# sunwookim028/bwa-mem-gpu

Hardware: AMD Instinct MI355X
Metric: reads/s aligned (150 bp PE vs hg38-scale 3100 Mbp synthetic genome), file to file (bwahip_stream_run) (higher is better)
Workload: dtype u64

## Files before the change

### bwa-mem-gpu_amd/bwahip.py

```python
import ctypes as C
import os
import subprocess
import numpy as np

_HERE = os.path.dirname(os.path.abspath(__file__))
LIB_PATH = os.environ.get("BWAHIP_LIB") or os.path.join(_HERE, "libbwahip.so")
TOOLS = os.path.join(_HERE, "tools")


class Opt(C.Structure):
    _fields_ = [("max_mem_intv", C.c_uint64), ("a", C.c_int), ("b", C.c_int), ("o_del", C.c_int), ("e_del", C.c_int),
                ("o_ins", C.c_int), ("e_ins", C.c_int), ("pen_unpaired", C.c_int), ("pen_clip5", C.c_int),
                ("pen_clip3", C.c_int), ("w", C.c_int), ("zdrop", C.c_int), ("T", C.c_int), ("flag", C.c_int),
                ("min_seed_len", C.c_int), ("min_chain_weight", C.c_int), ("max_chain_extend", C.c_int),
                ("split_factor", C.c_float), ("split_width", C.c_int), ("max_occ", C.c_int), ("max_chain_gap", C.c_int),
                ("n_threads", C.c_int), ("chunk_size", C.c_int), ("mask_level", C.c_float), ("drop_ratio", C.c_float),
                ("XA_drop_ratio", C.c_float), ("mask_level_redun", C.c_float), ("mapQ_coef_len", C.c_float),
                ("mapQ_coef_fac", C.c_int), ("max_ins", C.c_int), ("max_matesw", C.c_int), ("max_XA_hits", C.c_int),
                ("max_XA_hits_alt", C.c_int), ("mat", C.c_int8 * 25)]


class Seq(C.Structure):
    _fields_ = [("l_seq", C.c_int), ("id", C.c_int), ("name", C.c_char_p), ("comment", C.c_char_p),
                ("seq", C.POINTER(C.c_char)), ("qual", C.c_char_p), ("sam", C.POINTER(C.c_char)),
# ... 1149 lines not shown
        return ["k_smem(passes 1-2)+k_smem_heavy+k_smem3(pass 3)+k_intv_sort", "k_seeds", "k_chain(+k_chain_big,k_chain_flt)", "k_seed_sw (only with -W / reads > 700 bp)",
                "k_extend_spec+k_extend(+k_extend_big, dedup/patch)", "pe_rescue = PE: k_pestat + k_pe_prepare + k_pe_copy (insert sizes, lists; the rescue kernels k_matesw_sw / k_matesw start on the second stream)",
                "k_mark (mark primary) + PE: k_pair (pairing) beside the rescue kernels, then both for the rescued pairs",
                "k_cigar (mem_reg2aln: mapQ, CIGAR by ksw_global2 backtrack, NM/MD)", "k_sam size + scan + write (SAM text)"]

    @staticmethod
    def output_description(paired):
        return "SAM text of the batch in HBM (== seqs[i].sam of mem_process_seqs, " + ("paired-end: mate rescue, pairing, paired records)" if paired else "single-end)")

    def counters(self):
        buf = (C.c_uint64 * 32)()
        _check(lib().bwahip_batch_counters(self._h, buf, 32), "bwahip_batch_counters")
        names = ["extend", "blocks", "sa", "lf", "intv", "seeds", "cells", "max_extends", "chain_build_max", "chain_sort_max", "chain_flt_max",
                 "chain_write_max", "max_seeds", "max_chains", "ext_max", "ext_dedup_max", "heavy_blocks", "heavy_intv", "heavy_reads",
                 "dp_rows_1col", "dp_rows_ncol", "dedup_sort1_max", "dedup_loop_max", "dedup_sort2_max",
                 "pass3_blocks", "pass3_intv", "pass3_jumped", "ext_calls", "ext_diag", "_29", "_30", "_31"]
        return {k: int(buf[i]) for i, k in enumerate(names)}

    def kat_introsort(self, k64, score, qb, mode):
        k64 = np.ascontiguousarray(k64, dtype=np.int64); score = np.ascontiguousarray(score, dtype=np.int32); qb = np.ascontiguousarray(qb, dtype=np.int32)
        n = len(k64)
        a = np.empty(n, dtype=np.int32); b = np.empty(n, dtype=np.int32); st = np.zeros(2, dtype=np.int32)
        _check(lib().bwahip_kat_introsort(self._h, n, mode, k64.ctypes.data, score.ctypes.data, qb.ctypes.data, a.ctypes.data, b.ctypes.data, st.ctypes.data), "bwahip_kat_introsort")
        assert st[1] == 0
        return a, b, bool(st[0])

    def kat_mate_insert(self, list_off, list_words, step_off, step_hit, step_words, opt=None, mode=0, where=0):
        opt = opt or default_opt()
        list_off = np.ascontiguousarray(list_off, dtype=np.int64); step_off = np.ascontiguousarray(step_off, dtype=np.int64)
        list_words = np.ascontiguousarray(list_words, dtype=np.int64).reshape(-1, 19); step_words = np.ascontiguousarray(step_words, dtype=np.int64).reshape(-1, 19)
        step_hit = np.ascontiguousarray(step_hit, dtype=np.int32)
# ... 311 lines not shown
```

### bwa-mem-gpu_amd/csrc/bwahip_internal.h

```cpp
#pragma once
#include <hip/hip_runtime.h>
#include <stdint.h>
#include <stdio.h>
#include <stdlib.h>
#include <string.h>
#include <vector>
#include <string>
#include "../../include/bwahip.h"

#define HIP_TRY(expr) do { hipError_t e_ = (expr); if (e_ != hipSuccess) { \
	fprintf(stderr, "[bwahip] %s failed at %s:%d: %s\n", #expr, __FILE__, __LINE__, hipGetErrorString(e_)); \
	return BWAHIP_ENODEV; } } while (0)

struct DevAnn { int64_t offset; int32_t len; int32_t is_alt; };

struct DevIndex {
	const uint4 *bwt;
	const uint64_t *sa;
	const uint8_t *pac;
	const DevAnn *anns;
	uint64_t primary, L2[5], seq_len, n_sa;
	int64_t l_pac;
	int sa_intv, sa_shift, n_seqs;
	const uint4 *kmer; int kmer_k;
// ... 1 lines not shown
__host__ __device__ inline uint64_t kmer_off(int L) { return (0x5555555555555555ull & ((1ull << 2 * L) - 1)) - 1; }

struct DevOpt {
	int a, b, o_del, e_del, o_ins, e_ins, pen_clip5, pen_clip3, w, zdrop;
	int min_seed_len, split_width, max_occ, max_chain_gap, max_mem_intv, split_len;
	int min_chain_weight, max_chain_extend;
	float mask_level, drop_ratio, mask_level_redun;
	int8_t mat[25];
	int T, flag, pen_unpaired, max_ins, max_matesw, max_XA_hits, max_XA_hits_alt, mapQ_coef_fac;
	float XA_drop_ratio, mapQ_coef_len;
};

enum { CNT_EXTEND = 0, CNT_BLOCKS, CNT_SA, CNT_LF, CNT_INTV, CNT_SEEDS, CNT_CELLS, CNT_MAX_EXT ,
       CNT_HEAVY_BLOCKS = 16, CNT_HEAVY_INTV, CNT_HEAVY_READS, CNT_ROWS1 , CNT_ROWSN ,
       CNT_P3_BLOCKS = 24, CNT_P3_INTV, CNT_P3_JUMPED ,
       CNT_EXT_CALLS , CNT_EXT_DIAG , CNT_N = 32 };
constexpr int CNT_SLOTS = 256;
#define BWAHIP_MISC_BYTES ((size_t)CNT_SLOTS * CNT_N * 8 + 64)
#ifdef __HIPCC__
__device__ __forceinline__ unsigned long long *cnt_row(unsigned long long *base)
{
	return base + (size_t)((blockIdx.x * (blockDim.x >> 6) + (threadIdx.x >> 6)) & (CNT_SLOTS - 1)) * CNT_N;
}
#endif

struct __attribute__((aligned(32))) DevIntv { uint64_t x0, x1, x2, info; };

struct __attribute__((aligned(16))) DevSeed { int64_t rbeg; int32_t qbeg, len; int32_t score, rid; };

struct DevChain {
	int64_t pos;
// ... 36 lines not shown
	DevIndex ix; DevOpt opt;
	int n_reads; const uint8_t *seq; const int64_t *off;
	uint64_t *seq4; int seq4_stride;
	DevIntv *out; int *out_n; int cap;
	DevIntv *raw; int *raw_n;
	int *seed_cnt;
	float *frac_rep_lrep;
	int *l_rep;
	DevIntv *scratch; int lcap;
	unsigned int *queue;
	unsigned long long *counters;
	int *err;
	int groups_total;
	int *worst_n;
	int *heavy_list; unsigned int *heavy_n; int heavy_mult;
};
int launch_smem(const SmemLaunch &a, int group_lanes, hipStream_t st);
int launch_pack4(const SmemLaunch &a, hipStream_t st);
int launch_smem_heavy(const SmemLaunch &a, hipStream_t st);
int launch_smem3(const SmemLaunch &a, hipStream_t st);
int launch_kmer_table(const DevIndex &ix, uint4 *tab, int K, hipStream_t st);
int launch_kmer_check(const DevIndex &ix, int L, unsigned long long *bad, hipStream_t st);
int launch_intv_sort(const SmemLaunch &a, hipStream_t st);
int smem_default_groups(int group_lanes);

struct SeedLaunch {
	DevIndex ix; DevOpt opt;
	int n_reads; const int64_t *off;
	const DevIntv *intv; const int *intv_n; int cap;
	const int64_t *seed_base;
// ... 204 lines not shown
```

### bwa-mem-gpu_amd/csrc/ctx_internal.h

```cpp
#pragma once
#include "bwahip_internal.h"
#include "own.h"
#include <atomic>
#include <memory>
#include <string>
#include <utility>

inline std::atomic<long> g_bwahip_reallocs{0};
inline std::atomic<int64_t> g_bwahip_live[6];

struct DevMem {
	static constexpr size_t slack = 256;
	static constexpr const char *what = "hipMalloc";
	static void *alloc(size_t bytes)
	{
		void *p = nullptr;
		if (hipMalloc(&p, bytes ? bytes : 1) != hipSuccess) { (void)hipGetLastError(); return nullptr; }
		++g_bwahip_live[0]; g_bwahip_live[1] += (int64_t)bytes;
		return p;
	}
	static void free(void *p, size_t bytes) { (void)hipFree(p); --g_bwahip_live[0]; g_bwahip_live[1] -= (int64_t)bytes; }
	static void count_sync() { ++g_bwahip_reallocs; }
};
struct PinnedMem {
// ... 38 lines not shown
	{
		reset();
		if (hipStreamCreateWithFlags(&s, flags) != hipSuccess) { (void)hipGetLastError(); s = nullptr; return BWAHIP_ENODEV; }
		++g_bwahip_live[5];
		return 0;
	}
	void reset() { if (s) { (void)hipStreamDestroy(s); --g_bwahip_live[5]; s = nullptr; } }
	operator hipStream_t() const { return s; }
};

struct Knobs {
	int intv_cap = 96;
	int smem_lanes = 1;
	int sa_intv = 1;
	int kmer_k = 14;
	int heavy_mult = -1;
	int chain_mid_max = 1536, chain_big_max = 3200, chain_glb_grid = 2048;
	int chain_big_min = 512;
	int rank_sort_min = 2;
	int spec_min_chains = 16;
	int ext_lds_window = 1 << 30;
	int ext_early_stop = 1;
	int ext_diag = 1;
	int sorted_piece_blocks = 1024;
	int gpu_final = 1;
	int gpu_pair = 1;
	int incr_insert = 1;
	int verbose = 0;
	int e2e_log = 0;
	const char *dump_ext = nullptr;
	void from_env()
	{
		auto geti = [](const char *k, int &v) { if (const char *e = getenv(k)) v = atoi(e); };
		geti("BWAHIP_INTV_CAP", intv_cap); geti("BWAHIP_SMEM_LANES", smem_lanes); geti("BWAHIP_HEAVY_MULT", heavy_mult); geti("BWAHIP_SA_INTV", sa_intv); geti("BWAHIP_KMER_K", kmer_k);
		geti("BWAHIP_CHAIN_BIG_MIN", chain_big_min); geti("BWAHIP_CHAIN_MID_MAX", chain_mid_max); geti("BWAHIP_CHAIN_BIG_MAX", chain_big_max); geti("BWAHIP_CHAIN_GLB_GRID", chain_glb_grid); geti("BWAHIP_RANK_SORT_MIN", rank_sort_min); geti("BWAHIP_SPEC_MIN_CHAINS", spec_min_chains); geti("BWAHIP_EXT_LDS_WINDOW", ext_lds_window); geti("BWAHIP_EXT_EARLY_STOP", ext_early_stop); geti("BWAHIP_EXT_DIAG", ext_diag); geti("BWAHIP_GPU_FINAL", gpu_final); geti("BWAHIP_GPU_PAIR", gpu_pair);
		verbose = getenv("BWAHIP_VERBOSE") != nullptr;
		e2e_log = getenv("BWAHIP_E2E_LOG") != nullptr;
		dump_ext = getenv("BWAHIP_DUMP_EXT");
		if (intv_cap < 2) intv_cap = 2;
		ext_early_stop = ext_early_stop != 0; ext_diag = ext_diag != 0;
		geti("BWAHIP_INCR_INSERT", incr_insert); incr_insert = incr_insert != 0;
		geti("BWAHIP_SORTED_PIECE_BLOCKS", sorted_piece_blocks);
		if (sorted_piece_blocks < 1 || sorted_piece_blocks > 4096) sorted_piece_blocks = 1024;
	}
};

struct BatchText {
	std::vector<int64_t> off, qoff, noff, coff;
	int64_t qtot = 0;
// ... 200 lines not shown
```

### bwa-mem-gpu_amd/csrc/fmi_dev.h

```cpp
#pragma once
#include "bwahip_internal.h"

__device__ __forceinline__ int lane_id() { return (int)(threadIdx.x & 63); }

template <int K> __device__ __forceinline__ uint32_t quad_bcast(uint32_t v)
{
	constexpr int ctrl = K | K << 2 | K << 4 | K << 6;
	return (uint32_t)__builtin_amdgcn_update_dpp(0, (int)v, ctrl, 0xf, 0xf, false);
}
template <int K> __device__ __forceinline__ uint64_t quad_bcast64(uint64_t v)
{
	return (uint64_t)quad_bcast<K>((uint32_t)v) | (uint64_t)quad_bcast<K>((uint32_t)(v >> 32)) << 32;
}
__device__ __forceinline__ uint32_t quad_xor1(uint32_t v) { return (uint32_t)__builtin_amdgcn_update_dpp(0, (int)v, 0xB1, 0xf, 0xf, false); }
__device__ __forceinline__ uint32_t quad_xor2(uint32_t v) { return (uint32_t)__builtin_amdgcn_update_dpp(0, (int)v, 0x4E, 0xf, 0xf, false); }
__device__ __forceinline__ uint32_t half_mirror(uint32_t v) { return (uint32_t)__builtin_amdgcn_update_dpp(0, (int)v, 0x141, 0xf, 0xf, false); }
__device__ __forceinline__ uint64_t half_mirror64(uint64_t v)
{
	return (uint64_t)half_mirror((uint32_t)v) | (uint64_t)half_mirror((uint32_t)(v >> 32)) << 32;
}

__device__ __forceinline__ uint32_t count_bases64(uint4 v, int n)
{
	const int n0 = n < 32 ? n : 32, n1 = n - n0;
// ... 127 lines not shown
	const bool none = (p == ~0ull);
	uint64_t pp = p - (p >= ix.primary);
	uint4 v0 = make_uint4(0, 0, 0, 0), v1 = v0, v2 = v0, v3 = v0;
	if (live && !none) {
		const uint4 *b = ix.bwt + (pp >> 7) * 4;
		v0 = b[0]; v1 = b[1]; v2 = b[2]; v3 = b[3];
	}
	const int o = (int)(pp & 127) + 1;
	const uint32_t packed = count_bases64(v2, o < 64 ? o : 64) + count_bases64(v3, o > 64 ? o - 64 : 0);
	cnt[0] = ((uint64_t)v0.y << 32 | v0.x) + (packed & 0xff);
	cnt[1] = ((uint64_t)v0.w << 32 | v0.z) + (packed >> 8 & 0xff);
	cnt[2] = ((uint64_t)v1.y << 32 | v1.x) + (packed >> 16 & 0xff);
	cnt[3] = ((uint64_t)v1.w << 32 | v1.z) + (packed >> 24);
	if (none) cnt[0] = cnt[1] = cnt[2] = cnt[3] = 0;
}
__device__ __forceinline__ void lane_occ4_pair(const DevIndex &ix, uint64_t pk, uint64_t pl, bool live, uint64_t ck[4], uint64_t cl[4])
{
	const bool nk = (pk == ~0ull);
	const uint64_t kk = pk - (pk >= ix.primary), ll = pl - (pl >= ix.primary);
	uint4 a0 = make_uint4(0, 0, 0, 0), a1 = a0, a2 = a0, a3 = a0;
	const bool same = !nk && (kk >> 7) == (ll >> 7);
	const bool k_hi = (kk & 127) >= 64, l_hi = (ll & 127) >= 64;
	if (live && !nk) { const uint4 *b = ix.bwt + (kk >> 7) * 4; a0 = b[0]; a1 = b[1]; a2 = b[2]; if (k_hi || (same && l_hi)) a3 = b[3]; }
	uint4 b0 = a0, b1 = a1, b2 = a2, b3 = a3;
	if (live && !same && pl != ~0ull) { const uint4 *b = ix.bwt + (ll >> 7) * 4; b0 = b[0]; b1 = b[1]; b2 = b[2]; if (l_hi) b3 = b[3]; }
	{
		const int o = (int)(kk & 127) + 1;
		const uint32_t packed = count_bases64(a2, o < 64 ? o : 64) + count_bases64(a3, o > 64 ? o - 64 : 0);
		ck[0] = ((uint64_t)a0.y << 32 | a0.x) + (packed & 0xff); ck[1] = ((uint64_t)a0.w << 32 | a0.z) + (packed >> 8 & 0xff);
		ck[2] = ((uint64_t)a1.y << 32 | a1.x) + (packed >> 16 & 0xff); ck[3] = ((uint64_t)a1.w << 32 | a1.z) + (packed >> 24);
		if (nk) ck[0] = ck[1] = ck[2] = ck[3] = 0;
	}
	{
		const int o = (int)(ll & 127) + 1;
		const uint32_t packed = count_bases64(b2, o < 64 ? o : 64) + count_bases64(b3, o > 64 ? o - 64 : 0);
		cl[0] = ((uint64_t)b0.y << 32 | b0.x) + (packed & 0xff); cl[1] = ((uint64_t)b0.w << 32 | b0.z) + (packed >> 8 & 0xff);
		cl[2] = ((uint64_t)b1.y << 32 | b1.x) + (packed >> 16 & 0xff); cl[3] = ((uint64_t)b1.w << 32 | b1.z) + (packed >> 24);
		if (pl == ~0ull) cl[0] = cl[1] = cl[2] = cl[3] = 0;
	}
}

__device__ __forceinline__ int lane_extend_c(const DevIndex &ix, const Bi &ik, int is_back, int c, bool live, Bi &o)
{
	uint64_t xa = is_back ? ik.x0 : ik.x1;
	uint64_t xb = is_back ? ik.x1 : ik.x0;
	uint64_t k = xa - 1, l = k + ik.x2;
	uint64_t tk[4], tl[4];
	lane_occ4_pair(ix, k, l, live, tk, tl);
	uint64_t s1 = tl[1] - tk[1], s2 = tl[2] - tk[2], s3 = tl[3] - tk[3];
	uint64_t lo = L2_at(ix, c) + 1 + sel4(c, tk[0], tk[1], tk[2], tk[3]);
	uint64_t sz = sel4(c, tl[0] - tk[0], s1, s2, s3);
	uint64_t cum = (c < 3 ? s3 : 0) + (c < 2 ? s2 : 0) + (c < 1 ? s1 : 0);
	uint64_t bb = xb + (xa <= ix.primary && xa + ik.x2 - 1 >= ix.primary) + cum;
	o.x0 = is_back ? lo : bb;
	o.x1 = is_back ? bb : lo;
	o.x2 = sz;
	if (!live) return 0;
	uint64_t kk = k - (k >= ix.primary), ll = l - (l >= ix.primary);
	return (k == ~0ull || (kk >> 7) != (ll >> 7)) ? 2 : 1;
}

__device__ __forceinline__ uint64_t pair_swap64(uint64_t v) { return (uint64_t)quad_xor1((uint32_t)v) | (uint64_t)quad_xor1((uint32_t)(v >> 32)) << 32; }
__device__ __forceinline__ int pair_extend_c(const DevIndex &ix, const Bi &ik, int is_back, int c, bool live, Bi &o)
// ... 68 lines not shown
```

### bwa-mem-gpu_amd/csrc/k_smem.hip

```cpp
#include "fmi_dev.h"

namespace {

enum : int { ST_IDLE = 0, ST_NEXT, ST_FWD, ST_BWD, ST_FINISH };

__device__ __forceinline__ void put(DevIntv *p, uint64_t x0, uint64_t x1, uint64_t x2, uint64_t info)
{
	ulonglong2 *q = reinterpret_cast<ulonglong2*>(p);
	q[0] = make_ulonglong2(x0, x1);
	q[1] = make_ulonglong2(x2, info);
}
__device__ __forceinline__ void get(const DevIntv *p, uint64_t &x0, uint64_t &x1, uint64_t &x2, uint64_t &info)
{
	const ulonglong2 *q = reinterpret_cast<const ulonglong2*>(p);
	ulonglong2 a = q[0], b = q[1];
	x0 = a.x; x1 = a.y; x2 = b.x; info = b.y;
}

__device__ __forceinline__ uint64_t get_info(const DevIntv *p) { return reinterpret_cast<const ulonglong2*>(p)[1].y; }
__device__ __forceinline__ uint64_t get_x2(const DevIntv *p) { return reinterpret_cast<const ulonglong2*>(p)[1].x; }

__device__ __forceinline__ uint4 pack_entry(uint64_t x0, uint64_t x1, uint64_t x2, uint32_t end)
{
	const uint32_t h0 = (uint32_t)(x0 >> 32), h1 = (uint32_t)(x1 >> 32), h2 = (uint32_t)(x2 >> 32);
// ... 1 lines not shown
}
__device__ __forceinline__ void unpack_entry(uint4 v, uint64_t &x0, uint64_t &x1, uint64_t &x2, uint64_t &end)
{
	x0 = (uint64_t)(v.w & 63) << 32 | v.x;
	x1 = (uint64_t)(v.w >> 6 & 63) << 32 | v.y;
	x2 = (uint64_t)(v.w >> 12 & 63) << 32 | v.z;
	end = v.w >> 18;
}

__device__ __forceinline__ int qbase(const uint64_t *row, int p, uint64_t &qw, int &qwi)
{
	const int wi = p >> 4;
	if (wi != qwi) { qw = row[wi]; qwi = wi; }
	const uint32_t half = (p & 8) ? (uint32_t)(qw >> 32) : (uint32_t)qw;
	return (int)(half >> ((p & 7) * 4)) & 15;
}

__global__ __launch_bounds__(256) void k_pack4(int n_reads, const uint8_t *seq, const int64_t *off, uint64_t *seq4, int stride)
{
	const int64_t t = (int64_t)blockIdx.x * blockDim.x + threadIdx.x;
	if (t >= (int64_t)n_reads * stride) return;
	const int r = (int)(t / stride), w = (int)(t % stride);
	const uint8_t *s = seq + off[r];
	const int len = (int)(off[r + 1] - off[r]);
	uint64_t v = 0;
	for (int k = 0; k < 16; ++k) {
		const int p = w * 16 + k;
		const uint64_t code = p < len ? (s[p] > 3 ? 4 : s[p]) : 15;
		v |= code << (4 * k);
	}
// ... 19 lines not shown
		if (x2 > (uint64_t)a.opt.max_occ) { uint64_t step = x2 / a.opt.max_occ; cnt = (x2 + step - 1) / step; }
		n_seed += (int)(cnt < (uint64_t)a.opt.max_occ ? cnt : (uint64_t)a.opt.max_occ);
	}
	for (int m = 32; m; m >>= 1) n_seed += __shfl_xor(n_seed, m);
	if (lane == 0) {
		a.out_n[rd] = n_emit;
		a.seed_cnt[rd] = n_emit > cap ? 0 : n_seed;
		if (n_emit > cap) atomicMax(a.worst_n, n_emit);
	}
}

__device__ __forceinline__ void finish_pass12(const SmemLaunch &a, int rd, int n_emit, int n_ext)
{
	a.raw_n[rd] = n_emit;
	a.l_rep[rd] = n_ext;
	if ((unsigned long long)n_ext > cnt_row(a.counters)[CNT_MAX_EXT]) atomicMax(&cnt_row(a.counters)[CNT_MAX_EXT], (unsigned long long)n_ext);
}

__device__ __forceinline__ int base_or_minus1(int b) { return b > 3 ? -1 : b; }

__global__ __launch_bounds__(256) void k_kmer_level(DevIndex ix, uint4 *tab, int L)
{
	const uint64_t stride = (uint64_t)gridDim.x * blockDim.x;
	if (L == 1) {
		const int c = (int)(blockIdx.x * blockDim.x + threadIdx.x);
		if (c < 4) { Bi ik; set_intv(ix, c, ik); tab[kmer_off(1) + c] = pack_entry(ik.x0, ik.x1, ik.x2, 0); }
		return;
	}
	const uint64_t n_par = 1ull << 2 * (L - 1);
	const uint4 *par = tab + kmer_off(L - 1);
	uint4 *out = tab + kmer_off(L);
// ... 24 lines not shown
		const bool live = pre.x2 != 0;
		lane_extend_c(ix, pre, 0, 3 - last, live, o);
		const bool ok = live ? (o.x2 == got.x2 && (o.x2 == 0 || (o.x0 == got.x0 && o.x1 == got.x1))) : got.x2 == 0;
		if (!ok) atomicAdd(bad, 1ull);
	}
}

template <int G>
__global__ __launch_bounds__(256, 4) void k_smem(SmemLaunch a)
{
	const int lane = lane_id();
	const int gl = lane & (G - 1);
	const int group = (int)((blockIdx.x * blockDim.x + threadIdx.x) / G);
	const DevIndex &ix = a.ix;
	const int min_seed_len = a.opt.min_seed_len, cap = a.cap, lcap = a.lcap;

	constexpr int LL = 8 * G;
	__shared__ uint4 lds_list[(256 / G) * (LL + 1)];
	uint4 *const lrow = lds_list + (threadIdx.x / G) * (LL + 1);
	uint4 *const spill = reinterpret_cast<uint4*>(a.scratch) + (size_t)group * lcap;
	DevIntv *U = a.raw;

	int st = ST_IDLE, rd = -1, len = 0, pass = 0;
	const uint64_t *qrow = nullptr; uint64_t qw = 0; int qwi = -1;
	int x = 0, i = 0, j = 0, c = 0, min_intv = 1, ret = 0, p2k = 0, old_n = 0, out_n = 0;
	int prev_n = 0, curr_n = 0, base = 0, top = 0, mem_n = 0, mem_last_start = 0;
	uint64_t curr_last_x2 = 0, p_info = 0;
	Bi ik = { 0, 0, 0 };
	uint32_t ik_end = 0, last_push_end = 0;
	int guard = 0, guard_max = 0;
	bool exhausted = false;
	unsigned int n_ext = 0, n_blk = 0, n_out = 0;

#define LDS_SLOT(P) ((P) & (LL - 1))
#define LIST_PUT(P, X0, X1, X2, END) do { \
		const int p_ = (P); const uint4 v_ = pack_entry((X0), (X1), (X2), (uint32_t)(END)); \
		if (p_ >= top - LL) { if (gl == 0) lrow[LDS_SLOT(p_)] = v_; } else spill[p_] = v_; } while (0)
#define LIST_GET(P, X0, X1, X2, END) do { \
		const int p_ = (P); \
		uint4 v_ = lrow[LDS_SLOT(p_)]; \
		asm volatile("" : "+v"(v_.x), "+v"(v_.y), "+v"(v_.z), "+v"(v_.w)); \
		if (p_ < top - LL) v_ = spill[p_]; \
		unpack_entry(v_, (X0), (X1), (X2), (END)); } while (0)
#define PREV_AT(jj) (base + prev_n - 1 - (jj))
#define FWD_PUSH(X0, X1, X2, END) do { \
		const int p_ = curr_n; const uint4 v_ = pack_entry((X0), (X1), (X2), (uint32_t)(END)); \
		if (p_ >= LL) { uint4 ev_ = lrow[LDS_SLOT(p_)]; asm volatile("" : "+v"(ev_.x), "+v"(ev_.y), "+v"(ev_.z), "+v"(ev_.w)); spill[p_ - LL] = ev_; } \
		if (gl == 0) lrow[LDS_SLOT(p_)] = v_; \
		++curr_n; curr_last_x2 = (X2); } while (0)
#define BWD_PUSH(X0, X1, X2, END) do { LIST_PUT(PREV_AT(curr_n), (X0), (X1), (X2), (END)); ++curr_n; curr_last_x2 = (X2); } while (0)
#define EMIT(X0, X1, X2, INFO) do { if (out_n < cap) put(U + out_n, (X0), (X1), (X2), (INFO)); ++out_n; } while (0)
#define FOUND_MEM(X0, X1, X2, FWD_END, START) do { \
		if (mem_n == 0 || (START) < mem_last_start) { \
			++mem_n; mem_last_start = (START); \
			if ((int)(uint32_t)(FWD_END) - (START) >= min_seed_len) EMIT((X0), (X1), (X2), (uint64_t)(START) << 32 | (uint32_t)(FWD_END)); \
		} } while (0)
#define QB(p) qbase(qrow, (p), qw, qwi)
#define BASE_AT(p) ((p) < 0 ? -1 : base_or_minus1(QB(p)))
#define START_SMEM(X_, MI) do { \
		x = (X_); min_intv = (MI) < 1 ? 1 : (MI); \
		mem_n = 0; curr_n = 0; base = 0; curr_last_x2 = 0; \
		set_intv(ix, QB(x), ik); ik_end = (uint32_t)(x + 1); i = x + 1; st = ST_FWD; } while (0)
#define FWD_FINISH() do { \
		ret = (int)last_push_end; \
		__builtin_amdgcn_wave_barrier(); \
		prev_n = curr_n; top = curr_n; base = 0; curr_n = 0; \
		i = x - 1; j = 0; c = BASE_AT(i); st = ST_BWD; } while (0)
#define BWD_FINISH() do { st = ST_NEXT; if (pass == 1) x = ret; } while (0)

	for (;;) {
		if (st == ST_IDLE && !exhausted) {
			unsigned t = 0;
			if (gl == 0) t = atomicAdd(a.queue, 1u);
			if (G > 1) t = __shfl(t, lane & ~(G - 1));
			if (t >= (unsigned)a.n_reads) exhausted = true;
			else {
				rd = (int)t; qrow = a.seq4 + (size_t)t * a.seq4_stride; qwi = -1; U = a.raw + (size_t)t * cap; len = (int)(a.off[t + 1] - a.off[t]);
				out_n = 0; pass = 1; x = 0; guard = 0;
				guard_max = a.heavy_mult > 0 ? a.heavy_mult * len + 64 : 64 * BWAHIP_MAX_READ_LEN;
				st = len < min_seed_len ? ST_FINISH : ST_NEXT;
			}
		}
		if (__ballot(st != ST_IDLE) == 0) break;

		bool need = false; int is_back = 0, cb = 0; Bi req = { 0, 0, 0 };
		for (int spin = 0; spin < 8192 && !need && st != ST_IDLE && st != ST_FINISH; ++spin) {
			if (st == ST_NEXT) {
				if (pass == 1) {
					while (x < len && QB(x) > 3) ++x;
					if (x < len) START_SMEM(x, 1);
					else { pass = 2; old_n = out_n < cap ? out_n : cap; p2k = 0; }
				} else if (pass == 2) {
					bool started = false;
					while (p2k < old_n && !started) {
						uint64_t x0, x1, x2, info;
						get(U + p2k, x0, x1, x2, info); ++p2k;
						int b = (int)(info >> 32), e = (int)(uint32_t)info;
						if (e - b < a.opt.split_len || x2 > (uint64_t)a.opt.split_width) continue;
						if (QB((b + e) >> 1) > 3) continue;
						START_SMEM((b + e) >> 1, (int)x2 + 1);
						started = true;
					}
					if (!started) st = ST_FINISH;
				}
			}
			if (st == ST_FWD) {
				const int bq = i < len ? QB(i) : 4;
				if (bq < 4) { need = true; is_back = 0; req = ik; cb = 3 - bq; }
				else {
					FWD_PUSH(ik.x0, ik.x1, ik.x2, ik_end); last_push_end = ik_end;
					FWD_FINISH();
				}
			}
			if (st == ST_BWD && !need) {
				if (c < 0) {
					for (int jj = 0; jj < prev_n; ++jj) {
						uint64_t x0, x1, x2, info;
						LIST_GET(PREV_AT(jj), x0, x1, x2, info);
						FOUND_MEM(x0, x1, x2, info, i + 1);
					}
					BWD_FINISH();
				} else {
					LIST_GET(PREV_AT(j), req.x0, req.x1, req.x2, p_info);
					need = true; is_back = 1; cb = c;
				}
			}
		}

		if (st == ST_FINISH) {
			if (gl == 0) { finish_pass12(a, rd, out_n, guard); n_out += out_n < cap ? out_n : cap; }
			st = ST_IDLE; rd = -1;
		}

		Bi o;
		const bool live = need;
		int nb = G == 8 ? group8_extend_c(ix, req, is_back, cb, live, o) : G == 4 ? quad_extend_c(ix, req, is_back, cb, live, o) : G == 2 ? pair_extend_c(ix, req, is_back, cb, live, o)
		                                                                        : lane_extend_c(ix, req, is_back, cb, live, o);
		if (need && gl == 0) { ++n_ext; n_blk += nb; }

		if (need) {
			if (++guard > guard_max) {
				if (a.heavy_mult > 0) {
					if (gl == 0) { unsigned h = atomicAdd(a.heavy_n, 1u); a.heavy_list[h] = rd; }
					st = ST_IDLE; rd = -1;
				} else {
					if (gl == 0) atomicExch(a.err, 1);
					out_n = 0; st = ST_FINISH;
				}
			} else if (st == ST_FWD) {
				bool stop = false;
				if (o.x2 != ik.x2) {
					FWD_PUSH(ik.x0, ik.x1, ik.x2, ik_end); last_push_end = ik_end;
					if (o.x2 < (uint64_t)min_intv) stop = true;
				}
				if (stop) FWD_FINISH();
				else { ik = o; ik_end = (uint32_t)(i + 1); ++i; }
			} else if (st == ST_BWD) {
				if (o.x2 < (uint64_t)min_intv) {
					if (curr_n == 0) FOUND_MEM(req.x0, req.x1, req.x2, p_info, i + 1);
				} else if (curr_n == 0 || o.x2 != curr_last_x2) {
					BWD_PUSH(o.x0, o.x1, o.x2, p_info);
				}
				if (++j == prev_n) {
					if (curr_n == 0) BWD_FINISH();
					else {
						__builtin_amdgcn_wave_barrier();
						base += prev_n - curr_n; prev_n = curr_n; curr_n = 0;
						--i; j = 0; c = BASE_AT(i);
					}
				}
			}
		}
	}
	{
		unsigned long long e = gl == 0 ? n_ext : 0, b = gl == 0 ? n_blk : 0, o = gl == 0 ? n_out : 0;
		for (int m = 32; m; m >>= 1) { e += __shfl_xor(e, m); b += __shfl_xor(b, m); o += __shfl_xor(o, m); }
		if (lane == 0 && (e | o)) {
			unsigned long long *cnt = cnt_row(a.counters);
			atomicAdd(&cnt[CNT_EXTEND], e); atomicAdd(&cnt[CNT_BLOCKS], b); atomicAdd(&cnt[CNT_INTV], o);
		}
	}
#undef PREV_AT
#undef FWD_PUSH
#undef BWD_PUSH
#undef LIST_PUT
#undef LIST_GET
#undef LDS_SLOT
#undef EMIT
#undef FOUND_MEM
#undef BASE_AT
#undef QB
#undef START_SMEM
#undef FWD_FINISH
#undef BWD_FINISH
}

struct HeavyRead {
	const uint64_t *qrow; int len;
	uint4 *L; DevIntv *U;
	int out_n, ext;
	uint64_t qw; int qwi;
	unsigned n_ext, n_blk;
};

__device__ __forceinline__ void heavy_emit(const SmemLaunch &a, HeavyRead &r, int lane, uint64_t x0, uint64_t x1, uint64_t x2, uint64_t info)
{
	if (r.out_n < a.cap && lane == 0) put(r.U + r.out_n, x0, x1, x2, info);
	++r.out_n;
}
// ... 282 lines not shown
```

### bwa-mem-gpu_amd/csrc/runtime.hip

```cpp
#include "ctx_internal.h"
#include <math.h>
#include <algorithm>
#include <atomic>

namespace {
constexpr int SCAN_T = 256, SCAN_PER = 16, SCAN_TILE = SCAN_T * SCAN_PER;

__device__ __forceinline__ long long block_excl_scan(long long v, long long *sh, long long *total)
{
	const int t = threadIdx.x;
	sh[t] = v;
	__syncthreads();
	for (int d = 1; d < SCAN_T; d <<= 1) {
		long long o = t >= d ? sh[t - d] : 0;
		__syncthreads();
		sh[t] += o;
		__syncthreads();
	}
	const long long incl = sh[t];
	*total = sh[SCAN_T - 1];
	__syncthreads();
	return incl - v;
}

// ... 318 lines not shown
}

int bwahip_ctx_set_rg_id(bwahip_ctx *c, const char *id) { if (!c) return BWAHIP_EINVAL; c->rg_id = id ? id : ""; return 0; }
const char *bwahip_ctx_rg_id(const bwahip_ctx *c) { return c ? c->rg_id.c_str() : ""; }
const bwahip_bns_t *bwahip_bns(const bwahip_ctx *c) { return c ? &c->host.bns : nullptr; }
const bwahip_bwt_t *bwahip_bwt(const bwahip_ctx *c) { return c ? &c->host.bwt : nullptr; }
const uint8_t *bwahip_pac(const bwahip_ctx *c) { return c ? c->host.pac : nullptr; }

int bwahip_ctx_tune(bwahip_ctx *c, const char *key, int value)
{
	if (!c || !key) return BWAHIP_EINVAL;
	Knobs &k = c->knobs;
	if (!strcmp(key, "intv_cap")) { k.intv_cap = value < 2 ? 2 : value; c->intv_cap = k.intv_cap; }
	else if (!strcmp(key, "smem_lanes")) { if (value != 1 && value != 2 && value != 4 && value != 8) return BWAHIP_EINVAL; k.smem_lanes = value; }
	else if (!strcmp(key, "heavy_mult")) k.heavy_mult = value;
	else if (!strcmp(key, "chain_big_min")) k.chain_big_min = value;
	else if (!strcmp(key, "chain_mid_max")) k.chain_mid_max = value;
	else if (!strcmp(key, "chain_big_max")) k.chain_big_max = value;
	else if (!strcmp(key, "chain_glb_grid")) { if (value < 1 || value > 65536) return BWAHIP_EINVAL; k.chain_glb_grid = value; }
	else if (!strcmp(key, "rank_sort_min")) k.rank_sort_min = value;
	else if (!strcmp(key, "spec_min_chains")) k.spec_min_chains = value;
	else if (!strcmp(key, "ext_lds_window")) k.ext_lds_window = value < 1 ? 1 : value;
	else if (!strcmp(key, "ext_early_stop")) { if (value != 0 && value != 1) return BWAHIP_EINVAL; k.ext_early_stop = value; }
	else if (!strcmp(key, "ext_diag")) { if (value != 0 && value != 1) return BWAHIP_EINVAL; k.ext_diag = value; }
	else if (!strcmp(key, "sorted_piece_blocks")) { if (value < 1 || value > 4096) return BWAHIP_EINVAL; k.sorted_piece_blocks = value; }
	else if (!strcmp(key, "gpu_final")) k.gpu_final = value;
	else if (!strcmp(key, "gpu_pair")) k.gpu_pair = value;
	else if (!strcmp(key, "incr_insert")) { if (value != 0 && value != 1) return BWAHIP_EINVAL; k.incr_insert = value; }
	else if (!strcmp(key, "verbose")) k.verbose = value;
	else return BWAHIP_EINVAL;
// ... 295 lines not shown
	HIP_TRY(hipMemsetAsync(c->d_redo.p, 0, 16, c->stream));
	if ((rc = c->d_dedup.ensure(((size_t)3 * n + 4) * 4))) return rc;
	HIP_TRY(hipMemsetAsync(c->d_dedup.p, 0, 16, c->stream));
	el.dedup_n = c->d_dedup.as<int>(); el.dedup_list = c->d_dedup.as<int>() + 4;
	el.redo_n = c->d_redo.as<int>(); el.redo_list = c->d_redo.as<int>() + 4; el.big_t = c->d_big_t.as<uint8_t>(); el.lds_window = c->knobs.ext_lds_window; el.ext_early_stop = c->knobs.ext_early_stop; el.ext_diag = c->knobs.ext_diag;
	el.rank_sort_min = c->knobs.rank_sort_min;
	const int spec_min = c->knobs.spec_min_chains;
	if (spec_min > 0) {
		if ((rc = c->d_spec_regs.ensure(T * sizeof(DevReg))) || (rc = c->d_spec_items.ensure(T * 8 + 16))) return rc;
		el.spec_regs = c->d_spec_regs.as<DevReg>(); el.spec_n = c->d_spec_items.as<int>(); el.spec_items = (int2*)(c->d_spec_items.as<int>() + 4);
		el.spec_min_chains = spec_min;
	}
	return 0;
}

int run_pipeline(bwahip_ctx *c, const bwahip_opt_t *opt, bool timed, bool dump)
{
	const bool verbose = c->knobs.verbose != 0;
#define STAGE_LOG(name) do { if (verbose) { (void)hipStreamSynchronize(c->stream); fprintf(stderr, "[bwahip] %s done (%s)\n", name, hipGetErrorString(hipGetLastError())); fflush(stderr); } } while (0)
	const int n = c->in->n;
	if (n == 0) return 0;
	DevOpt dopt = make_dev_opt(opt);
	if (c->ix.seq_len >= (1ull << 38) || c->in->max_len >= (1 << 14)) return BWAHIP_EINVAL;
	unsigned long long *counters = c->d_misc.as<unsigned long long>();
	unsigned int *queue = (unsigned int*)(counters + (size_t)CNT_SLOTS * CNT_N);
	int *err = (int*)(queue + 4);
	int rc;
	for (int attempt = 0; attempt < 8; ++attempt) {
		const int cap = c->intv_cap, lcap = c->in->max_len + 2;
		const int G = c->knobs.smem_lanes;
// ... 5 lines not shown
		HIP_TRY(hipMemsetAsync(c->d_misc.p, 0, BWAHIP_MISC_BYTES, c->stream));
		SmemLaunch sl;
		memset(&sl, 0, sizeof sl);
		sl.ix = c->ix; sl.opt = dopt; sl.n_reads = n; sl.seq = c->in->d_seq.as<uint8_t>(); sl.off = c->in->d_off.as<int64_t>();
		sl.out = c->d_intv.as<DevIntv>(); sl.out_n = c->d_intv_n.as<int>(); sl.cap = cap;
		sl.raw = c->d_raw.as<DevIntv>(); sl.raw_n = c->d_raw_n.as<int>();
		sl.seed_cnt = c->d_seed_cnt.as<int>(); sl.l_rep = c->d_lrep.as<int>();
		sl.seq4_stride = (c->in->max_len + 15) / 16 + 1;
		if ((rc = c->d_seq4.ensure((size_t)n * sl.seq4_stride * 8))) return rc;
		sl.seq4 = c->d_seq4.as<uint64_t>();
		if (attempt == 0 && (rc = launch_pack4(sl, c->stream))) return rc;
		sl.scratch = c->d_scratch.as<DevIntv>(); sl.lcap = lcap; sl.queue = queue; sl.counters = counters; sl.err = err; sl.groups_total = groups;
		const int heavy_mult = c->knobs.heavy_mult >= 0 ? c->knobs.heavy_mult : c->in->max_len <= 200 ? 10 : 30;
		if ((rc = c->d_smem_heavy.ensure((size_t)n * 4))) return rc;
		sl.heavy_list = c->d_smem_heavy.as<int>(); sl.heavy_n = queue + 1; sl.heavy_mult = heavy_mult; sl.worst_n = (int*)(queue + 2);
		if (timed) HIP_TRY(hipEventRecord(c->ev[0], c->stream));
		if ((rc = launch_smem(sl, G, c->stream))) return rc;
		STAGE_LOG("k_smem");
		if (timed) HIP_TRY(hipEventRecord(c->ev[1], c->stream));
		if (heavy_mult > 0 && (rc = launch_smem_heavy(sl, c->stream))) return rc;
		STAGE_LOG("k_smem_heavy");
		if (timed) HIP_TRY(hipEventRecord(c->ev[12], c->stream));
		if ((rc = launch_smem3(sl, c->stream))) return rc;
		STAGE_LOG("k_smem3");
		if (timed) HIP_TRY(hipEventRecord(c->ev[13], c->stream));
		if ((rc = launch_intv_sort(sl, c->stream))) return rc;
		STAGE_LOG("k_intv_sort");
		if (timed) HIP_TRY(hipEventRecord(c->ev[10], c->stream));
		if ((rc = launch_scan(c->d_seed_cnt.as<int>(), c->d_seed_base.as<int64_t>(), n, c->d_scan, c->stream))) return rc;
		if (timed) HIP_TRY(hipEventRecord(c->ev[2], c->stream));
// ... 687 lines not shown
```

Baseline: 12.90 million.

## Jump SMEM search over first J bases via k-mer interval table

In the single-lane SMEM kernel, each forward search now starts by looking up the first J bases in the precomputed k-mer interval table, replacing J backward-extension BWT occurrence lookups with one table load. The backward phase likewise uses a table lookup when it reaches the last J bases. If the jumped interval is too small, the read's output for that start is rolled back and the plain step-by-step search runs instead. Per-thread counters move to shared-memory atomics, and two new counters record table lookups and fallbacks. The cost is extra state-machine complexity and some wasted work when a jump falls back.

Measured after the change: 14.44 million, median of 6. 11.9% higher.

```diff
diff --git a/bwa-mem-gpu_amd/bwahip.py b/bwa-mem-gpu_amd/bwahip.py
--- a/bwa-mem-gpu_amd/bwahip.py
+++ b/bwa-mem-gpu_amd/bwahip.py
@@ -1187,7 +1187,7 @@
         names = ["extend", "blocks", "sa", "lf", "intv", "seeds", "cells", "max_extends", "chain_build_max", "chain_sort_max", "chain_flt_max",
                  "chain_write_max", "max_seeds", "max_chains", "ext_max", "ext_dedup_max", "heavy_blocks", "heavy_intv", "heavy_reads",
                  "dp_rows_1col", "dp_rows_ncol", "dedup_sort1_max", "dedup_loop_max", "dedup_sort2_max",
-                 "pass3_blocks", "pass3_intv", "pass3_jumped", "ext_calls", "ext_diag", "_29", "_30", "_31"]
+                 "pass3_blocks", "pass3_intv", "pass3_jumped", "ext_calls", "ext_diag", "smem_lookups", "smem_fallbacks", "_31"]
         return {k: int(buf[i]) for i, k in enumerate(names)}
 
     def kat_introsort(self, k64, score, qb, mode):
diff --git a/bwa-mem-gpu_amd/csrc/bwahip_internal.h b/bwa-mem-gpu_amd/csrc/bwahip_internal.h
--- a/bwa-mem-gpu_amd/csrc/bwahip_internal.h
+++ b/bwa-mem-gpu_amd/csrc/bwahip_internal.h
@@ -39,7 +39,8 @@
 enum { CNT_EXTEND = 0, CNT_BLOCKS, CNT_SA, CNT_LF, CNT_INTV, CNT_SEEDS, CNT_CELLS, CNT_MAX_EXT ,
        CNT_HEAVY_BLOCKS = 16, CNT_HEAVY_INTV, CNT_HEAVY_READS, CNT_ROWS1 , CNT_ROWSN ,
        CNT_P3_BLOCKS = 24, CNT_P3_INTV, CNT_P3_JUMPED ,
-       CNT_EXT_CALLS , CNT_EXT_DIAG , CNT_N = 32 };
+       CNT_EXT_CALLS , CNT_EXT_DIAG ,
+       CNT_SMEM_LOOKUPS , CNT_SMEM_FALLBACKS , CNT_N = 32 };
 constexpr int CNT_SLOTS = 256;
 #define BWAHIP_MISC_BYTES ((size_t)CNT_SLOTS * CNT_N * 8 + 64)
 #ifdef __HIPCC__
@@ -106,6 +107,7 @@
 	int groups_total;
 	int *worst_n;
 	int *heavy_list; unsigned int *heavy_n; int heavy_mult;
+	int smem_skip;
 };
 int launch_smem(const SmemLaunch &a, int group_lanes, hipStream_t st);
 int launch_pack4(const SmemLaunch &a, hipStream_t st);
diff --git a/bwa-mem-gpu_amd/csrc/ctx_internal.h b/bwa-mem-gpu_amd/csrc/ctx_internal.h
--- a/bwa-mem-gpu_amd/csrc/ctx_internal.h
+++ b/bwa-mem-gpu_amd/csrc/ctx_internal.h
@@ -76,6 +76,7 @@
 	int smem_lanes = 1;
 	int sa_intv = 1;
 	int kmer_k = 14;
+	int smem_skip = -1;
 	int heavy_mult = -1;
 	int chain_mid_max = 1536, chain_big_max = 3200, chain_glb_grid = 2048;
 	int chain_big_min = 512;
@@ -94,7 +95,7 @@
 	void from_env()
 	{
 		auto geti = [](const char *k, int &v) { if (const char *e = getenv(k)) v = atoi(e); };
-		geti("BWAHIP_INTV_CAP", intv_cap); geti("BWAHIP_SMEM_LANES", smem_lanes); geti("BWAHIP_HEAVY_MULT", heavy_mult); geti("BWAHIP_SA_INTV", sa_intv); geti("BWAHIP_KMER_K", kmer_k);
+		geti("BWAHIP_INTV_CAP", intv_cap); geti("BWAHIP_SMEM_LANES", smem_lanes); geti("BWAHIP_HEAVY_MULT", heavy_mult); geti("BWAHIP_SMEM_SKIP", smem_skip); geti("BWAHIP_SA_INTV", sa_intv); geti("BWAHIP_KMER_K", kmer_k);
 		geti("BWAHIP_CHAIN_BIG_MIN", chain_big_min); geti("BWAHIP_CHAIN_MID_MAX", chain_mid_max); geti("BWAHIP_CHAIN_BIG_MAX", chain_big_max); geti("BWAHIP_CHAIN_GLB_GRID", chain_glb_grid); geti("BWAHIP_RANK_SORT_MIN", rank_sort_min); geti("BWAHIP_SPEC_MIN_CHAINS", spec_min_chains); geti("BWAHIP_EXT_LDS_WINDOW", ext_lds_window); geti("BWAHIP_EXT_EARLY_STOP", ext_early_stop); geti("BWAHIP_EXT_DIAG", ext_diag); geti("BWAHIP_GPU_FINAL", gpu_final); geti("BWAHIP_GPU_PAIR", gpu_pair);
 		verbose = getenv("BWAHIP_VERBOSE") != nullptr;
 		e2e_log = getenv("BWAHIP_E2E_LOG") != nullptr;
diff --git a/bwa-mem-gpu_amd/csrc/fmi_dev.h b/bwa-mem-gpu_amd/csrc/fmi_dev.h
--- a/bwa-mem-gpu_amd/csrc/fmi_dev.h
+++ b/bwa-mem-gpu_amd/csrc/fmi_dev.h
@@ -165,13 +165,21 @@
 	cnt[3] = ((uint64_t)v1.w << 32 | v1.z) + (packed >> 24);
 	if (none) cnt[0] = cnt[1] = cnt[2] = cnt[3] = 0;
 }
-__device__ __forceinline__ void lane_occ4_pair(const DevIndex &ix, uint64_t pk, uint64_t pl, bool live, uint64_t ck[4], uint64_t cl[4])
+__device__ __forceinline__ void lane_occ4_pair(const DevIndex &ix, uint64_t pk, uint64_t pl, bool live, uint64_t ck[4], uint64_t cl[4],
+                                               const uint4 *other = nullptr, uint4 *first = nullptr)
 {
 	const bool nk = (pk == ~0ull);
 	const uint64_t kk = pk - (pk >= ix.primary), ll = pl - (pl >= ix.primary);
 	uint4 a0 = make_uint4(0, 0, 0, 0), a1 = a0, a2 = a0, a3 = a0;
 	const bool same = !nk && (kk >> 7) == (ll >> 7);
 	const bool k_hi = (kk & 127) >= 64, l_hi = (ll & 127) >= 64;
+	if (first) {
+		const bool lk = live && !nk;
+		const uint4 *b = lk ? ix.bwt + (kk >> 7) * 4 : other;
+		if (lk || other) a0 = b[0];
+		if (lk) { a1 = b[1]; a2 = b[2]; if (k_hi || (same && l_hi)) a3 = b[3]; }
+		*first = a0;
+	} else
 	if (live && !nk) { const uint4 *b = ix.bwt + (kk >> 7) * 4; a0 = b[0]; a1 = b[1]; a2 = b[2]; if (k_hi || (same && l_hi)) a3 = b[3]; }
 	uint4 b0 = a0, b1 = a1, b2 = a2, b3 = a3;
 	if (live && !same && pl != ~0ull) { const uint4 *b = ix.bwt + (ll >> 7) * 4; b0 = b[0]; b1 = b[1]; b2 = b[2]; if (l_hi) b3 = b[3]; }
@@ -191,13 +199,13 @@
 	}
 }
 
-__device__ __forceinline__ int lane_extend_c(const DevIndex &ix, const Bi &ik, int is_back, int c, bool live, Bi &o)
+__device__ __forceinline__ int lane_extend_c(const DevIndex &ix, const Bi &ik, int is_back, int c, bool live, Bi &o, const uint4 *other = nullptr, uint4 *first = nullptr)
 {
 	uint64_t xa = is_back ? ik.x0 : ik.x1;
 	uint64_t xb = is_back ? ik.x1 : ik.x0;
 	uint64_t k = xa - 1, l = k + ik.x2;
 	uint64_t tk[4], tl[4];
-	lane_occ4_pair(ix, k, l, live, tk, tl);
+	lane_occ4_pair(ix, k, l, live, tk, tl, other, first);
 	uint64_t s1 = tl[1] - tk[1], s2 = tl[2] - tk[2], s3 = tl[3] - tk[3];
 	uint64_t lo = L2_at(ix, c) + 1 + sel4(c, tk[0], tk[1], tk[2], tk[3]);
 	uint64_t sz = sel4(c, tl[0] - tk[0], s1, s2, s3);
diff --git a/bwa-mem-gpu_amd/csrc/k_smem.hip b/bwa-mem-gpu_amd/csrc/k_smem.hip
--- a/bwa-mem-gpu_amd/csrc/k_smem.hip
+++ b/bwa-mem-gpu_amd/csrc/k_smem.hip
@@ -2,7 +2,7 @@
 
 namespace {
 
-enum : int { ST_IDLE = 0, ST_NEXT, ST_FWD, ST_BWD, ST_FINISH };
+enum : int { ST_IDLE = 0, ST_NEXT, ST_JUMP, ST_FWD, ST_BWD, ST_FINISH };
 
 __device__ __forceinline__ void put(DevIntv *p, uint64_t x0, uint64_t x1, uint64_t x2, uint64_t info)
 {
@@ -39,6 +39,22 @@
 	if (wi != qwi) { qw = row[wi]; qwi = wi; }
 	const uint32_t half = (p & 8) ? (uint32_t)(qw >> 32) : (uint32_t)qw;
 	return (int)(half >> ((p & 7) * 4)) & 15;
+}
+
+__device__ __forceinline__ bool kmer_code(const uint64_t *row, int x, int J, uint32_t &code)
+{
+	const int wi = x >> 4, sh = (x & 15) * 4;
+	const uint64_t w0 = row[wi], w1 = row[wi + 1];
+	uint64_t w = sh ? (w0 >> sh | w1 << (64 - sh)) : w0;
+	if (J < 16) w &= (1ull << 4 * J) - 1;
+	const bool acgt = (w & 0xCCCCCCCCCCCCCCCCull) == 0;
+	w = (w | w >> 2) & 0x0F0F0F0F0F0F0F0Full;
+	w = (w | w >> 4) & 0x00FF00FF00FF00FFull;
+	w = (w | w >> 8) & 0x0000FFFF0000FFFFull;
+	w = (w | w >> 16);
+	code = (uint32_t)w;
+	asm volatile("" : "+v"(code));
+	return acgt;
 }
 
 __global__ __launch_bounds__(256) void k_pack4(int n_reads, const uint8_t *seq, const int64_t *off, uint64_t *seq4, int stride)
@@ -88,7 +104,8 @@
 {
 	a.raw_n[rd] = n_emit;
 	a.l_rep[rd] = n_ext;
-	if ((unsigned long long)n_ext > cnt_row(a.counters)[CNT_MAX_EXT]) atomicMax(&cnt_row(a.counters)[CNT_MAX_EXT], (unsigned long long)n_ext);
+	unsigned long long *const mx = a.counters + (size_t)(rd & (CNT_SLOTS - 1)) * CNT_N + CNT_MAX_EXT;
+	if ((unsigned long long)n_ext > *mx) atomicMax(mx, (unsigned long long)n_ext);
 }
 
 __device__ __forceinline__ int base_or_minus1(int b) { return b > 3 ? -1 : b; }
@@ -143,23 +160,31 @@
 	const int group = (int)((blockIdx.x * blockDim.x + threadIdx.x) / G);
 	const DevIndex &ix = a.ix;
 	const int min_seed_len = a.opt.min_seed_len, cap = a.cap, lcap = a.lcap;
+	const int J = G == 1 ? a.smem_skip : 0;
+	const uint32_t jmask = J >= 16 ? ~0u : (1u << 2 * J) - 1;
+	const uint4 *const jtab = ix.kmer + kmer_off(J);
 
 	constexpr int LL = 8 * G;
 	__shared__ uint4 lds_list[(256 / G) * (LL + 1)];
 	uint4 *const lrow = lds_list + (threadIdx.x / G) * (LL + 1);
 	uint4 *const spill = reinterpret_cast<uint4*>(a.scratch) + (size_t)group * lcap;
 	DevIntv *U = a.raw;
+	__shared__ unsigned skip_cnt[4][4];
+	unsigned *const my_cnt = skip_cnt[threadIdx.x >> 6];
+	if (lane == 0) { my_cnt[0] = 0; my_cnt[1] = 0; my_cnt[2] = 0; my_cnt[3] = 0; }
+	__builtin_amdgcn_fence(__ATOMIC_RELEASE, "wavefront"); __builtin_amdgcn_wave_barrier(); __builtin_amdgcn_fence(__ATOMIC_ACQUIRE, "wavefront");
 
 	int st = ST_IDLE, rd = -1, len = 0, pass = 0;
 	const uint64_t *qrow = nullptr; uint64_t qw = 0; int qwi = -1;
 	int x = 0, i = 0, j = 0, c = 0, min_intv = 1, ret = 0, p2k = 0, old_n = 0, out_n = 0;
-	int prev_n = 0, curr_n = 0, base = 0, top = 0, mem_n = 0, mem_last_start = 0;
-	uint64_t curr_last_x2 = 0, p_info = 0;
+	int prev_n = 0, curr_n = 0, base = 0, top = 0, mem_last_start = 0;
+	uint64_t curr_last_x2 = 0; uint32_t p_info = 0;
 	Bi ik = { 0, 0, 0 };
 	uint32_t ik_end = 0, last_push_end = 0;
-	int guard = 0, guard_max = 0;
+	int guard = 0;
+	int dorm = 0;
 	bool exhausted = false;
-	unsigned int n_ext = 0, n_blk = 0, n_out = 0;
+	unsigned int n_blk = 0;
 
 #define LDS_SLOT(P) ((P) & (LL - 1))
 #define LIST_PUT(P, X0, X1, X2, END) do { \
@@ -173,27 +198,37 @@
 		unpack_entry(v_, (X0), (X1), (X2), (END)); } while (0)
 #define PREV_AT(jj) (base + prev_n - 1 - (jj))
 #define FWD_PUSH(X0, X1, X2, END) do { \
-		const int p_ = curr_n; const uint4 v_ = pack_entry((X0), (X1), (X2), (uint32_t)(END)); \
+		const int p_ = base + curr_n; const uint4 v_ = pack_entry((X0), (X1), (X2), (uint32_t)(END)); \
 		if (p_ >= LL) { uint4 ev_ = lrow[LDS_SLOT(p_)]; asm volatile("" : "+v"(ev_.x), "+v"(ev_.y), "+v"(ev_.z), "+v"(ev_.w)); spill[p_ - LL] = ev_; } \
 		if (gl == 0) lrow[LDS_SLOT(p_)] = v_; \
 		++curr_n; curr_last_x2 = (X2); } while (0)
 #define BWD_PUSH(X0, X1, X2, END) do { LIST_PUT(PREV_AT(curr_n), (X0), (X1), (X2), (END)); ++curr_n; curr_last_x2 = (X2); } while (0)
 #define EMIT(X0, X1, X2, INFO) do { if (out_n < cap) put(U + out_n, (X0), (X1), (X2), (INFO)); ++out_n; } while (0)
 #define FOUND_MEM(X0, X1, X2, FWD_END, START) do { \
-		if (mem_n == 0 || (START) < mem_last_start) { \
-			++mem_n; mem_last_start = (START); \
+		if ((START) < mem_last_start) { \
+			mem_last_start = (START); \
 			if ((int)(uint32_t)(FWD_END) - (START) >= min_seed_len) EMIT((X0), (X1), (X2), (uint64_t)(START) << 32 | (uint32_t)(FWD_END)); \
 		} } while (0)
 #define QB(p) qbase(qrow, (p), qw, qwi)
 #define BASE_AT(p) ((p) < 0 ? -1 : base_or_minus1(QB(p)))
 #define START_SMEM(X_, MI) do { \
 		x = (X_); min_intv = (MI) < 1 ? 1 : (MI); \
-		mem_n = 0; curr_n = 0; base = 0; curr_last_x2 = 0; \
-		set_intv(ix, QB(x), ik); ik_end = (uint32_t)(x + 1); i = x + 1; st = ST_FWD; } while (0)
+		mem_last_start = 0x7fffffff; curr_n = 0; curr_last_x2 = 0; \
+		uint32_t code_ = 0; \
+		const bool jump_ = J && dorm >= 0 && kmer_code(qrow, x, J, code_); \
+		if (jump_) { lrow[LL].y = code_; dorm = J - 1; base = J - 1; ik_end = (uint32_t)(x + J); i = x + J; st = ST_JUMP; lrow[LL].x = (uint32_t)out_n; } \
+		else { dorm = 0; base = 0; set_intv(ix, QB(x), ik); ik_end = (uint32_t)(x + 1); i = x + 1; st = ST_FWD; } } while (0)
+#define ABANDON() do { \
+		out_n = (int)lrow[LL].x; dorm = -1; if (pass == 2) --p2k; st = ST_NEXT; \
+		if (gl == 0) __hip_atomic_fetch_add(&my_cnt[1], 1u, __ATOMIC_RELAXED, __HIP_MEMORY_SCOPE_WORKGROUP); } while (0)
+#define BWD_SWAP() do { \
+		__builtin_amdgcn_wave_barrier(); \
+		base += prev_n - curr_n; prev_n = curr_n; curr_n = 0; \
+		--i; j = 0; c = BASE_AT(i); } while (0)
 #define FWD_FINISH() do { \
 		ret = (int)last_push_end; \
 		__builtin_amdgcn_wave_barrier(); \
-		prev_n = curr_n; top = curr_n; base = 0; curr_n = 0; \
+		prev_n = curr_n; top = base + curr_n; curr_n = 0; \
 		i = x - 1; j = 0; c = BASE_AT(i); st = ST_BWD; } while (0)
 #define BWD_FINISH() do { st = ST_NEXT; if (pass == 1) x = ret; } while (0)
 
@@ -206,13 +241,12 @@
 			else {
 				rd = (int)t; qrow = a.seq4 + (size_t)t * a.seq4_stride; qwi = -1; U = a.raw + (size_t)t * cap; len = (int)(a.off[t + 1] - a.off[t]);
 				out_n = 0; pass = 1; x = 0; guard = 0;
-				guard_max = a.heavy_mult > 0 ? a.heavy_mult * len + 64 : 64 * BWAHIP_MAX_READ_LEN;
 				st = len < min_seed_len ? ST_FINISH : ST_NEXT;
 			}
 		}
 		if (__ballot(st != ST_IDLE) == 0) break;
 
-		bool need = false; int is_back = 0, cb = 0; Bi req = { 0, 0, 0 };
+		bool need = false, is_tab = false; int is_back = 0, cb = 0; Bi req = { 0, 0, 0 };
 		for (int spin = 0; spin < 8192 && !need && st != ST_IDLE && st != ST_FINISH; ++spin) {
 			if (st == ST_NEXT) {
 				if (pass == 1) {
@@ -233,6 +267,7 @@
 					if (!started) st = ST_FINISH;
 				}
 			}
+			if (J && st == ST_JUMP) { need = true; is_tab = true; }
 			if (st == ST_FWD) {
 				const int bq = i < len ? QB(i) : 4;
 				if (bq < 4) { need = true; is_back = 0; req = ik; cb = 3 - bq; }
@@ -249,33 +284,46 @@
 						FOUND_MEM(x0, x1, x2, info, i + 1);
 					}
 					BWD_FINISH();
+				} else if (J && j == prev_n) {
+					lrow[LL].y = (lrow[LL].y << 2 | (uint32_t)c) & jmask;
+					need = true; is_tab = true;
 				} else {
-					LIST_GET(PREV_AT(j), req.x0, req.x1, req.x2, p_info);
+					{ uint64_t e64_; LIST_GET(PREV_AT(j), req.x0, req.x1, req.x2, e64_); p_info = (uint32_t)e64_; }
 					need = true; is_back = 1; cb = c;
 				}
 			}
 		}
 
 		if (st == ST_FINISH) {
-			if (gl == 0) { finish_pass12(a, rd, out_n, guard); n_out += out_n < cap ? out_n : cap; }
+			if (gl == 0) { finish_pass12(a, rd, out_n, guard); __hip_atomic_fetch_add(&my_cnt[2], (unsigned)(out_n < cap ? out_n : cap), __ATOMIC_RELAXED, __HIP_MEMORY_SCOPE_WORKGROUP);
+				__hip_atomic_fetch_add(&my_cnt[3], (unsigned)guard, __ATOMIC_RELAXED, __HIP_MEMORY_SCOPE_WORKGROUP); }
 			st = ST_IDLE; rd = -1;
 		}
 
 		Bi o;
-		const bool live = need;
+		const bool live = need && !is_tab;
+		uint4 tv = make_uint4(0, 0, 0, 0);
 		int nb = G == 8 ? group8_extend_c(ix, req, is_back, cb, live, o) : G == 4 ? quad_extend_c(ix, req, is_back, cb, live, o) : G == 2 ? pair_extend_c(ix, req, is_back, cb, live, o)
-		                                                                        : lane_extend_c(ix, req, is_back, cb, live, o);
-		if (need && gl == 0) { ++n_ext; n_blk += nb; }
+		                                                                        : lane_extend_c(ix, req, is_back, cb, live, o, is_tab ? jtab + lrow[LL].y : nullptr, &tv);
+		if (live && gl == 0) n_blk += nb;
+		if (is_tab) {
+			uint64_t e_;
+			unpack_entry(tv, o.x0, o.x1, o.x2, e_);
+			if (gl == 0) __hip_atomic_fetch_add(&my_cnt[0], 1u, __ATOMIC_RELAXED, __HIP_MEMORY_SCOPE_WORKGROUP);
+		}
 
 		if (need) {
-			if (++guard > guard_max) {
+			if (++guard > (a.heavy_mult > 0 ? a.heavy_mult * len + 64 : 64 * BWAHIP_MAX_READ_LEN)) {
 				if (a.heavy_mult > 0) {
-					if (gl == 0) { unsigned h = atomicAdd(a.heavy_n, 1u); a.heavy_list[h] = rd; }
+					if (gl == 0) { unsigned h = atomicAdd(a.heavy_n, 1u); a.heavy_list[h] = rd; __hip_atomic_fetch_add(&my_cnt[3], (unsigned)guard, __ATOMIC_RELAXED, __HIP_MEMORY_SCOPE_WORKGROUP); }
 					st = ST_IDLE; rd = -1;
 				} else {
 					if (gl == 0) atomicExch(a.err, 1);
 					out_n = 0; st = ST_FINISH;
 				}
+			} else if (J && st == ST_JUMP) {
+				if (o.x2 < (uint64_t)min_intv) ABANDON();
+				else { ik = o; st = ST_FWD; }
 			} else if (st == ST_FWD) {
 				bool stop = false;
 				if (o.x2 != ik.x2) {
@@ -284,29 +332,41 @@
 				}
 				if (stop) FWD_FINISH();
 				else { ik = o; ik_end = (uint32_t)(i + 1); ++i; }
+			} else if (J && st == ST_BWD && is_tab) {
+				if (o.x2 < (uint64_t)min_intv) ABANDON();
+				else {
+					if (curr_n == 0 || o.x2 != curr_last_x2) BWD_PUSH(o.x0, o.x1, o.x2, (uint32_t)(i + J));
+					--dorm;
+					BWD_SWAP();
+				}
 			} else if (st == ST_BWD) {
 				if (o.x2 < (uint64_t)min_intv) {
 					if (curr_n == 0) FOUND_MEM(req.x0, req.x1, req.x2, p_info, i + 1);
 				} else if (curr_n == 0 || o.x2 != curr_last_x2) {
 					BWD_PUSH(o.x0, o.x1, o.x2, p_info);
 				}
-				if (++j == prev_n) {
+				if (++j == prev_n && dorm <= 0) {
 					if (curr_n == 0) BWD_FINISH();
-					else {
-						__builtin_amdgcn_wave_barrier();
-						base += prev_n - curr_n; prev_n = curr_n; curr_n = 0;
-						--i; j = 0; c = BASE_AT(i);
-					}
+					else BWD_SWAP();
 				}
 			}
 		}
 	}
 	{
-		unsigned long long e = gl == 0 ? n_ext : 0, b = gl == 0 ? n_blk : 0, o = gl == 0 ? n_out : 0;
-		for (int m = 32; m; m >>= 1) { e += __shfl_xor(e, m); b += __shfl_xor(b, m); o += __shfl_xor(o, m); }
-		if (lane == 0 && (e | o)) {
-			unsigned long long *cnt = cnt_row(a.counters);
-			atomicAdd(&cnt[CNT_EXTEND], e); atomicAdd(&cnt[CNT_BLOCKS], b); atomicAdd(&cnt[CNT_INTV], o);
+		unsigned long long b = gl == 0 ? n_blk : 0;
+		for (int m = 32; m; m >>= 1) b += __shfl_xor(b, m);
+		__builtin_amdgcn_fence(__ATOMIC_RELEASE, "wavefront"); __builtin_amdgcn_wave_barrier(); __builtin_amdgcn_fence(__ATOMIC_ACQUIRE, "wavefront");
+		if (lane == 0) {
+			const unsigned lk = __hip_atomic_load(&my_cnt[0], __ATOMIC_RELAXED, __HIP_MEMORY_SCOPE_WORKGROUP);
+			const unsigned fb = __hip_atomic_load(&my_cnt[1], __ATOMIC_RELAXED, __HIP_MEMORY_SCOPE_WORKGROUP);
+			const unsigned long long o = __hip_atomic_load(&my_cnt[2], __ATOMIC_RELAXED, __HIP_MEMORY_SCOPE_WORKGROUP);
+			const unsigned long long e = __hip_atomic_load(&my_cnt[3], __ATOMIC_RELAXED, __HIP_MEMORY_SCOPE_WORKGROUP) - lk;
+			unsigned wv = threadIdx.x >> 6;
+			asm volatile("" : "+v"(wv));
+			unsigned long long *cnt = a.counters + (size_t)((blockIdx.x * (blockDim.x >> 6) + wv) & (CNT_SLOTS - 1)) * CNT_N;
+			if (e | o) { atomicAdd(&cnt[CNT_EXTEND], e); atomicAdd(&cnt[CNT_BLOCKS], b); atomicAdd(&cnt[CNT_INTV], o); }
+			if (lk) atomicAdd(&cnt[CNT_SMEM_LOOKUPS], (unsigned long long)lk);
+			if (fb) atomicAdd(&cnt[CNT_SMEM_FALLBACKS], (unsigned long long)fb);
 		}
 	}
 #undef PREV_AT
@@ -322,6 +382,8 @@
 #undef START_SMEM
 #undef FWD_FINISH
 #undef BWD_FINISH
+#undef ABANDON
+#undef BWD_SWAP
 }
 
 struct HeavyRead {
diff --git a/bwa-mem-gpu_amd/csrc/runtime.hip b/bwa-mem-gpu_amd/csrc/runtime.hip
--- a/bwa-mem-gpu_amd/csrc/runtime.hip
+++ b/bwa-mem-gpu_amd/csrc/runtime.hip
@@ -356,6 +356,7 @@
 	if (!strcmp(key, "intv_cap")) { k.intv_cap = value < 2 ? 2 : value; c->intv_cap = k.intv_cap; }
 	else if (!strcmp(key, "smem_lanes")) { if (value != 1 && value != 2 && value != 4 && value != 8) return BWAHIP_EINVAL; k.smem_lanes = value; }
 	else if (!strcmp(key, "heavy_mult")) k.heavy_mult = value;
+	else if (!strcmp(key, "smem_skip")) { if (value < -1 || value == 1) return BWAHIP_EINVAL; k.smem_skip = value; }
 	else if (!strcmp(key, "chain_big_min")) k.chain_big_min = value;
 	else if (!strcmp(key, "chain_mid_max")) k.chain_mid_max = value;
 	else if (!strcmp(key, "chain_big_max")) k.chain_big_max = value;
@@ -681,6 +682,15 @@
 	return 0;
 }
 
+static int smem_skip_depth(const DevIndex &ix, int knob, int min_seed_len)
+{
+	int J = knob;
+	if (J < 0) for (J = 0; J < 16 && (1ull << 2 * (J + 1)) <= ix.seq_len / 16; ++J);
+	if (J > ix.kmer_k) J = ix.kmer_k;
+	if (J > min_seed_len) J = min_seed_len;
+	return J < 2 ? 0 : J;
+}
+
 int run_pipeline(bwahip_ctx *c, const bwahip_opt_t *opt, bool timed, bool dump)
 {
 	const bool verbose = c->knobs.verbose != 0;
@@ -716,6 +726,7 @@
 		const int heavy_mult = c->knobs.heavy_mult >= 0 ? c->knobs.heavy_mult : c->in->max_len <= 200 ? 10 : 30;
 		if ((rc = c->d_smem_heavy.ensure((size_t)n * 4))) return rc;
 		sl.heavy_list = c->d_smem_heavy.as<int>(); sl.heavy_n = queue + 1; sl.heavy_mult = heavy_mult; sl.worst_n = (int*)(queue + 2);
+		sl.smem_skip = smem_skip_depth(c->ix, c->knobs.smem_skip, dopt.min_seed_len);
 		if (timed) HIP_TRY(hipEventRecord(c->ev[0], c->stream));
 		if ((rc = launch_smem(sl, G, c->stream))) return rc;
 		STAGE_LOG("k_smem");
```
